# jglaser/metadynamics-plugin

Hardware: AMD Instinct MI355X
Metric: particle_cv_evals_per_s (higher is better)
Workload: dtype f32; 1 GPU; 1xMI355X: 10^6 particles, 2 lamellar CVs (8 Fourier modes each), 256^2 bias grid, well-tempered; particles_per_gpu=1000000, particles_global=1000000, n_cv=2, modes_per_cv=8, grid=256x256, stride=1, fast_trig=1, fast_trig_library_default=1, driver=host, mode=single

## Files before the change

### metadynamics-plugin_amd/csrc/fused.hip

```cpp
#include <hip/hip_runtime.h>
#include <hip/hip_ext.h>

#ifdef MTD_STAMPS
__device__ unsigned long long g_stamps[64];
#define MTD_STAMP(slot, cond)                                                   \
    do                                                                          \
        {                                                                       \
        if (cond) g_stamps[slot] = wall_clock64();                              \
        } while (0)
extern "C" int mtd_debug_read_stamps(unsigned long long *host)
    {
    return (int)hipMemcpyFromSymbol(host, HIP_SYMBOL(g_stamps), sizeof(unsigned long long) * 64);
    }
#else
#define MTD_STAMP(slot, cond) do { } while (0)
#endif

#include "lamellar_host.hpp"
#include "metad_host.hpp"
#include "comm_host.hpp"

#include <cstdlib>
#include <cstring>
#include <map>
// ... 181 lines not shown
        grid_first_pass_sums_256(c, blockIdx.x, sums, s_red);
        MTD_STAMP(20, blockIdx.x == 0 && threadIdx.x == 0);
        }
    else if (wave != 0 && N)
        {
        lam_force_store<S4, NCV, FF_U>(a, out, first, stride, s_wcoef, R);
        if (GROUPS > 1) lam_force_store<S4, NCV, FF_U>(a, out, first1, stride, s_wcoef, R1);
        MTD_STAMP(29, blockIdx.x == n_grid_blocks && threadIdx.x == 64);
        }

    if (blockIdx.x == 0 && wave == 0) publish_step(c, s_chain, deposit, nullptr, COMM ? &ck : nullptr);
    }

template<typename S4, bool FAST>
__global__ __launch_bounds__(FF_THREADS) void k_fused_force_general(const LamKArgs a, const S4 *__restrict__ postype, const ForcePtrs out,
                                                            const unsigned int N, const double two_over_n, const MetadCfg c,
                                                            const int deposit, const unsigned int n_grid_blocks)
    {
    __shared__ EvalShared sh;
    __shared__ float s_wcoef[MTD_MAX_CV * MTD_MAX_TYPES];
    __shared__ double s_red[16];
    __shared__ ModeTables s_mt;

    load_modes(a, s_mt, true);
    reduce_cv_sources(c, sh.cv, s_red);
    __syncthreads();
    evaluate_bias(c, sh, deposit != 0, true);

    if (blockIdx.x < n_grid_blocks)
        {
        const unsigned int g = blockIdx.x * FF_THREADS + threadIdx.x;
        double s1 = 0.0, s2 = 0.0;
        if (g < c.len)
            {
            const double dV = (c.W * sh.scal) * exp(-gauss_exponent(c, g, sh.cv));
            c.grid_delta[g] = dV;
            unsigned int hd = c.hist_delta[g];
            if (sh.on_grid && g == sh.bin)
                {
                hd += 1;
                c.hist_delta[g] = hd;
                c.sigma_grid_delta[g] += c.det_sigma;
                c.hist_gauss_delta[g] += 1;
                }
            const double R = c.rew[g] + (double)hd;
            c.rew[g] = R;
            s1 = R * dV;
// ... 173 lines not shown
    if (slots)
        {
        if (m->comm) return MTD_ERR_UNSUPPORTED;
        for (unsigned int c = 0; c < set->n_cv; ++c)
            {
            if (slots[c] >= m->cfg.n_cv) return MTD_ERR_INVALID_ARGUMENT;
            k.slot[c] = (unsigned char)slots[c];
            }
        }
    hipStream_t s = (hipStream_t)stream;
    rc = metad_flush(m, s);
    if (rc) return rc;
    ForcePtrs out;
    for (unsigned int c = 0; c < MTD_MAX_CV; ++c) out.f[c] = nullptr;
    for (unsigned int c = 0; c < set->n_cv; ++c)
        {
        if (!d_force[c] && n_particles) return MTD_ERR_INVALID_ARGUMENT;
        out.f[c] = d_force[c];
        }
    const int dep = deposit_due(m, timestep);
    const unsigned int n_grid = dep ? m->cfg.n_gblocks : 0;
    const double two_over_n = 2.0 / (double)n_global;
    const bool fast = lam_fast_trig(k) != 0;
    static const bool force_general = std::getenv("MTD_FUSED_GENERAL") != nullptr;
    CommK ck;
    std::memset(&ck, 0, sizeof(ck));
    if (m->comm)
        {
        if (m->cfg.n_cv > (unsigned int)CHAIN_MAX_CV || force_general) return MTD_ERR_UNSUPPORTED;
        rc = comm_current(m->comm, ck);
        if (rc) return rc;
        }
    if (m->cfg.n_cv <= (unsigned int)CHAIN_MAX_CV && !force_general)
        {
        hipEvent_t ev_start = nullptr, ev_stop = nullptr;
        const bool timed = force_profile_next(ev_start, ev_stop);
        dispatch_s4_fast(dtype, fast, [&](auto s4, auto fast_c)
            {
            using S4 = typename decltype(s4)::type;
            constexpr bool FAST = decltype(fast_c)::value;
            dispatch_count<CHAIN_MAX_CV>(set->n_cv, [&](auto n)
                {
                constexpr int NCV = decltype(n)::value, G = ff_groups<S4, NCV, FAST>::value;
                const unsigned int per_block = FF_STREAM_THREADS * FF_U * G;
                unsigned int fblocks = (n_particles + per_block - 1) / per_block;
                if (fblocks == 0 && n_grid == 0) fblocks = 1;
                const unsigned int grid = n_grid + fblocks;
                dispatch_bool(m->comm != nullptr, [&](auto comm_c)
                    {
                    dispatch_bool(k.ortho != 0, [&](auto ortho_c)
                        {
                        const auto kernel = k_fused_force<S4, NCV, FAST, G, decltype(comm_c)::value, decltype(ortho_c)::value>;
                        if (timed)
                            hipExtLaunchKernelGGL(kernel, dim3(grid), dim3(FF_THREADS), 0, s, ev_start, ev_stop, 0, k, (const S4 *)d_postype, out,
                                                  n_particles, two_over_n, m->cfg, dep, n_grid, ck);
                        else
                            kernel<<<grid, FF_THREADS, 0, s>>>(k, (const S4 *)d_postype, out, n_particles, two_over_n, m->cfg, dep, n_grid, ck);
                        });
                    });
                });
            });
        }
    else
        {
        unsigned int fblocks = lam_force_blocks(n_particles);
        if (n_particles == 0) fblocks = n_grid ? 0 : 1;
        const unsigned int grid = n_grid + fblocks;
        dispatch_s4_fast(dtype, fast, [&](auto s4, auto fast_c)
            {
            using S4 = typename decltype(s4)::type;
            k_fused_force_general<S4, decltype(fast_c)::value><<<grid, FF_THREADS, 0, s>>>(k, (const S4 *)d_postype, out, n_particles, two_over_n,
                                                                                        m->cfg, dep, n_grid);
            });
        }
    MTD_LAUNCH_CHECK();
    m->pending_apply = dep;
    m->w_stale = dep;
    return MTD_SUCCESS;
    }

int mtd_profile_force_begin(unsigned int n_launches)
    {
    std::lock_guard<std::mutex> lock(g_force_profile_mutex);
    ForceProfile &p = g_force_profile;
    for (hipEvent_t e : p.ev) (void)hipEventDestroy(e);
    p.ev.clear();
    p.used = 0;
    for (unsigned int i = 0; i < 2 * n_launches; ++i)
        {
        hipEvent_t e = nullptr;
        MTD_HIP_TRY(hipEventCreate(&e));
        p.ev.push_back(e);
        }
    return MTD_SUCCESS;
// ... 64 lines not shown
```

### metadynamics-plugin_amd/csrc/fused_step.hip

```cpp
#include <hip/hip_runtime.h>

#ifdef MTD_STAMPS
__device__ unsigned long long g_step_stamps[64];
__device__ unsigned long long g_step_block[6][256];
#define MTD_BSTAMP(row) do { g_step_block[row][blockIdx.x] = wall_clock64(); } while (0)
extern "C" int mtd_debug_read_step_blocks(unsigned long long *host)
    {
    return (int)hipMemcpyFromSymbol(host, HIP_SYMBOL(g_step_block), sizeof(unsigned long long) * 6 * 256);
    }
#define MTD_STAMP(slot, cond)                                                   \
    do                                                                          \
        {                                                                       \
        if (cond) g_step_stamps[slot] = wall_clock64();                         \
        } while (0)
extern "C" int mtd_debug_read_step_stamps(unsigned long long *host)
    {
    return (int)hipMemcpyFromSymbol(host, HIP_SYMBOL(g_step_stamps), sizeof(unsigned long long) * 64);
    }
#else
#define MTD_STAMP(slot, cond) do { } while (0)
#define MTD_BSTAMP(row) do { } while (0)
#endif

#include "lamellar_host.hpp"
#include "metad_host.hpp"
#include "comm_host.hpp"

#include <cstdlib>
#include <cstring>

namespace
{

using namespace mtd;

constexpr int FS_THREADS = 1024;
constexpr int FS_WAVES = FS_THREADS / MTD_WAVE;
constexpr int FS_U = 4;
constexpr unsigned int FS_MAX_BLOCKS = 256;
constexpr unsigned int FS_MAIN = (FS_WAVES - 1) * MTD_WAVE;
constexpr unsigned int FS_EXTRA_WAVES = 4;
constexpr unsigned int FS_CHUNK = FS_U * FS_MAIN + FS_EXTRA_WAVES * MTD_WAVE;
constexpr unsigned int FS_LL_WORDS = 2 * (CHAIN_MAX_CV + 2);
constexpr int FS_FIRST_PROBE_SLEEP = 12;
constexpr unsigned int FS_LL_PITCH = 512;
constexpr unsigned int FS_LL_REPLICAS = 8;
constexpr unsigned int FS_LL_REPLICA_WORDS = FS_LL_WORDS * FS_LL_PITCH;

template<int NCV, int U> struct StepRegs
    {
    v2f g0[U / 2], g1[U / 2], g2[U / 2];
    int type[U];
    bool ok[U];
    float f[U][NCV][3];
    };

template<int NCV, bool FAST, int U>
__device__ __forceinline__ void step_cv_sums(const LamKArgs &a, const float *s_coeff, const ModeTables &mt, const StepRegs<NCV, U> &R,
                                             float (&acc)[NCV])
    {
    constexpr int P = U / 2;
// ... 22 lines not shown
                    sum[q] += h.w * ((cs * cs) * 2.0f - (FAST ? 0.99999994f : 1.0f));
                    }
                }
#pragma unroll
            for (int u = 0; u < U; ++u)
                {
                const float w = R.ok[u] ? s_coeff[c * MTD_MAX_TYPES + R.type[u]] : 0.0f;
                acc[c] += w * sum[u / 2][u % 2];
                }
            }
        }
    }

template<int NCV, bool FAST, int U>
__device__ __forceinline__ void step_force_unscaled(const LamKArgs &a, const ModeTables &mt, StepRegs<NCV, U> &R)
    {
#pragma unroll
    for (int c = 0; c < NCV; ++c)
        {
#pragma unroll
        for (int u = 0; u < U; ++u) R.f[u][c][0] = R.f[u][c][1] = R.f[u][c][2] = 0.0f;
        if (c < (int)a.n_cv)
            {
            const unsigned int k1 = a.first[c + 1];
#pragma unroll 4
            for (unsigned int k = a.first[c]; k < k1; ++k)
                {
                const float4 h = mt.h[k];
                const float4 q = mt.q[k];
#pragma unroll
                for (int u = 0; u < U; ++u)
                    {
                    const float s = sin2pi<FAST>(h.x * R.g0[u / 2][u % 2] + h.y * R.g1[u / 2][u % 2] + h.z * R.g2[u / 2][u % 2]);
                    R.f[u][c][0] += q.x * s;
                    R.f[u][c][1] += q.y * s;
                    R.f[u][c][2] += q.z * s;
                    }
                }
            }
        }
    }

template<int NCV> struct ExtraRegs
    {
    float g0, g1, g2;
    int type;
    bool ok;
    float f[NCV][3];
    };

template<int NCV, bool FAST>
__device__ __forceinline__ void step_cv_sums_one(const LamKArgs &a, const float *s_coeff, const ModeTables &mt, const ExtraRegs<NCV> &X,
                                                 float (&acc)[NCV])
    {
#pragma unroll
    for (int c = 0; c < NCV; ++c)
        if (c < (int)a.n_cv)
            {
            float sum = 0.0f;
            const unsigned int k1 = a.first[c] + a.nact[c];
#pragma unroll 4
            for (unsigned int k = a.first[c]; k < k1; ++k)
                {
                const float4 h = mt.h[k];
                const float cs = cos2pi<FAST>(h.x * X.g0 + h.y * X.g1 + h.z * X.g2);
                sum += cs;
                sum += h.w * ((cs * cs) * 2.0f - (FAST ? 0.99999994f : 1.0f));
                }
            acc[c] += (X.ok ? s_coeff[c * MTD_MAX_TYPES + X.type] : 0.0f) * sum;
            }
    }

template<int NCV, bool FAST>
__device__ __forceinline__ void step_force_unscaled_one(const LamKArgs &a, const ModeTables &mt, ExtraRegs<NCV> &X)
    {
#pragma unroll
    for (int c = 0; c < NCV; ++c)
        {
        X.f[c][0] = X.f[c][1] = X.f[c][2] = 0.0f;
        if (c < (int)a.n_cv)
            {
            const unsigned int k1 = a.first[c + 1];
#pragma unroll 4
            for (unsigned int k = a.first[c]; k < k1; ++k)
                {
                const float4 h = mt.h[k];
                const float4 q = mt.q[k];
                const float sn = sin2pi<FAST>(h.x * X.g0 + h.y * X.g1 + h.z * X.g2);
                X.f[c][0] += q.x * sn;
                X.f[c][1] += q.y * sn;
                X.f[c][2] += q.z * sn;
                }
            }
        }
    }

template<typename S4, int NCV, bool FAST, bool COMM>
__global__ __launch_bounds__(FS_THREADS, 1) void k_fused_step(const LamKArgs a, const S4 *__restrict__ postype, const ForcePtrs out,
                                                           const unsigned int N, const unsigned int chunk, const double two_over_n,
                                                           const MetadCfg c, const int deposit, const unsigned int cells_per_block,
                                                           const CommK lk, const CommK ck)
    {
    typedef typename scalar4_traits<S4>::scalar scalar;
    constexpr int NS = NCV;
    __shared__ ChainResult s_chain;
    __shared__ float s_coeff[MTD_MAX_CV * MTD_MAX_TYPES];
    __shared__ float s_wcoef[MTD_MAX_CV * MTD_MAX_TYPES];
    __shared__ double s_wave[FS_WAVES * NCV];
    __shared__ double s_red[2 * FS_WAVES];
    __shared__ double s_avg[2];

    __shared__ ModeTables s_cvt;
    __shared__ ModeTables s_mt;

    const int wave = threadIdx.x >> 6;
// ... 13 lines not shown
    const unsigned int ix = p0 + FS_U * FS_MAIN + slot0;
    GridPatch patch;
    X.ok = false;
    if (wave == 0)
        {
#pragma unroll
        for (int u = 0; u < FS_U; ++u) R.ok[u] = false;
        patch = chain_prefetch(c);
        }
    else
        {
#pragma unroll
        for (int u = 0; u < FS_U; ++u)
            {
            const unsigned int i = p0 + u * FS_MAIN + slot0;
            R.ok[u] = i < p1;
            if (N) raw.v[u] = postype[R.ok[u] ? i : N - 1];
            }
        X.ok = has_extra && ix < p1;
        if (N && has_extra) raw_x = postype[X.ok ? ix : N - 1];
        }
    load_coeff(a, s_coeff);
    load_modes_cv(a, s_cvt);
    load_modes(a, s_mt, true);
    __syncthreads();

    MTD_STAMP(1, blockIdx.x == 0 && threadIdx.x == 0); MTD_STAMP(17, blockIdx.x == gridDim.x - 1 && threadIdx.x == 0); MTD_STAMP(33, blockIdx.x == 0 && threadIdx.x == 64);
    float acc[NCV];
#pragma unroll
    for (int i = 0; i < NCV; ++i) acc[i] = 0.0f;
    if (wave != 0)
        {
#pragma unroll
        for (int u = 0; u < FS_U; ++u)
            {
            float x0 = 0.0f, x1 = 0.0f, x2 = 0.0f;
            R.type[u] = 0;
            if (N)
                {
                const Particle p = scalar4_traits<S4>::unpack(raw.v[u]);
                project(a, p, x0, x1, x2);
                R.type[u] = p.type;
                }
            R.g0[u / 2][u % 2] = x0;
            R.g1[u / 2][u % 2] = x1;
            R.g2[u / 2][u % 2] = x2;
            }
// ... 391 lines not shown
```

### metadynamics-plugin_amd/csrc/lamellar.hip

```cpp
#include "lamellar_device.hpp"

#include <cmath>
#include <cstdlib>
#include <cstring>

#include "lamellar_host.hpp"

namespace
{

using namespace mtd;

constexpr int CV_THREADS = 512;
constexpr int CV_UNROLL = 4;
constexpr int FORCE_THREADS = 256;
constexpr int FORCE_UNROLL = 2;

int g_fast_trig = 1;

template<typename S4, int NCV, bool FAST>
__global__ __launch_bounds__(CV_THREADS) void k_lamellar_cv_partials(const LamKArgs a, const S4 *__restrict__ postype,
                                                                     const unsigned int N, double *__restrict__ partials)
    {
    __shared__ float s_coeff[MTD_MAX_CV * MTD_MAX_TYPES];
// ... 85 lines not shown
    double v = 0.0;
    unsigned int b = lane;
    for (; b + 7 * MTD_WAVE < n_partials; b += 8 * MTD_WAVE)
        {
        double t[8];
#pragma unroll
        for (int u = 0; u < 8; ++u) t[u] = partials[(size_t)(b + u * MTD_WAVE) * stride + c];
#pragma unroll
        for (int u = 0; u < 8; ++u) v += t[u];
        }
    for (; b < n_partials; b += MTD_WAVE) v += partials[(size_t)b * stride + c];
    v = wave_sum(v);
    if (lane == 0) out[c] = shift + scale * v;
    }

template<typename S4, bool FAST>
__global__ __launch_bounds__(FORCE_THREADS) void k_lamellar_forces(const LamKArgs a, const S4 *__restrict__ postype,
                                                                   const ForcePtrs out, const unsigned int N,
                                                                   const double *__restrict__ d_bias, const double bias_host,
                                                                   const double two_over_n)
    {
    __shared__ float s_wcoef[MTD_MAX_CV * MTD_MAX_TYPES];
    __shared__ ModeTables s_mt;
    load_modes(a, s_mt, true);
    for (unsigned int i = threadIdx.x; i < MTD_MAX_CV * MTD_MAX_TYPES; i += blockDim.x)
        {
        const unsigned int c = i / MTD_MAX_TYPES;
        double b = 0.0;
        if (c < a.n_cv) b = d_bias ? d_bias[c] : bias_host;
        s_wcoef[i] = (float)((double)a.coeff[c][i % MTD_MAX_TYPES] * b * two_over_n);
        }
    __syncthreads();
    lam_force_pass<S4, FAST, FORCE_UNROLL>(a, postype, out, N, blockIdx.x * blockDim.x + threadIdx.x,
                                           gridDim.x * blockDim.x, s_wcoef, s_mt);
    }


unsigned int env_uint(const char *name, unsigned int dflt)
    {
    const char *s = std::getenv(name);
    if (!s || !*s) return dflt;
    long v = std::strtol(s, nullptr, 10);
    return v > 0 ? (unsigned int)v : dflt;
    }

unsigned int cv_blocks(unsigned int N)
    {
// ... 34 lines not shown
    reciprocal_rows(*box, k.B);
    k.ortho = (k.B[0][1] == 0.0 && k.B[0][2] == 0.0 && k.B[1][0] == 0.0 && k.B[1][2] == 0.0 && k.B[2][0] == 0.0 && k.B[2][1] == 0.0)
                  ? 1u : 0u;
    k.n_cv = set->n_cv;
    k.n_modes = set->n_modes;
    k.n_types = set->n_types;
    if (set->trig_mode != MTD_TRIG_DEFAULT && set->trig_mode != MTD_TRIG_HARDWARE && set->trig_mode != MTD_TRIG_ACCURATE)
        return MTD_ERR_INVALID_ARGUMENT;
    k.trig = (unsigned int)set->trig_mode;
    for (unsigned int c = 0; c <= set->n_cv; ++c) k.first[c] = set->first[c];
    for (unsigned int c = 0; c < MTD_MAX_CV; ++c) k.slot[c] = (unsigned char)c;
    const double two_pi = 2.0 * M_PI;
    for (unsigned int m = 0; m < set->n_modes; ++m)
        for (int d = 0; d < 3; ++d)
            {
            const float hv = (float)set->hkl[m][d];
            const float qv = (float)(two_pi * (set->hkl[m][0] * k.B[0][d] + set->hkl[m][1] * k.B[1][d] + set->hkl[m][2] * k.B[2][d]));
            if (d == 0) { k.h[m].x = hv; k.q[m].x = qv; }
            if (d == 1) { k.h[m].y = hv; k.q[m].y = qv; }
            if (d == 2) { k.h[m].z = hv; k.q[m].z = qv; }
            }
    for (unsigned int c = 0; c < set->n_cv; ++c)
        for (unsigned int t = 0; t < set->n_types; ++t) k.coeff[c][t] = (float)set->coeff[c][t];
    static const bool fold = env_uint("MTD_LAM_FOLD_HARMONICS", 1) != 0;
    for (unsigned int c = 0; c < set->n_cv; ++c)
        {
        bool folded[MTD_MAX_MODES] = {false};
        for (unsigned int m = set->first[c]; fold && m < set->first[c + 1]; ++m)
            {
            if (folded[m] || k.h[m].w != 0.0f) continue;
            const int *hm = set->hkl[m];
            if (hm[0] == 0 && hm[1] == 0 && hm[2] == 0) continue;
            for (unsigned int j = set->first[c]; j < set->first[c + 1]; ++j)
                {
                const int *hj = set->hkl[j];
                if (j != m && !folded[j] && k.h[j].w == 0.0f && hj[0] == 2 * hm[0] && hj[1] == 2 * hm[1] && hj[2] == 2 * hm[2])
                    {
                    k.h[m].w = 1.0f;
                    folded[j] = true;
                    break;
                    }
                }
            }
        unsigned int n = 0;
        for (unsigned int m = set->first[c]; m < set->first[c + 1]; ++m)
            if (!folded[m]) k.corder[set->first[c] + n++] = (unsigned char)m;
        k.nact[c] = (unsigned char)n;
        for (unsigned int m = set->first[c]; m < set->first[c + 1]; ++m)
            if (folded[m]) k.corder[set->first[c] + n++] = (unsigned char)m;
        }
    return MTD_SUCCESS;
    }


unsigned int lam_cv_blocks(unsigned int N) { return cv_blocks(N); }
unsigned int lam_force_blocks(unsigned int N) { return force_blocks(N); }
int lam_fast_trig(const LamKArgs &k)
    {
    if (k.trig == MTD_TRIG_ACCURATE) return 0;
    if (k.trig == MTD_TRIG_DEFAULT && !g_fast_trig) return 0;
    for (unsigned int m = 0; m < k.n_modes; ++m)
        if (std::fabs(k.h[m].x) + std::fabs(k.h[m].y) + std::fabs(k.h[m].z) > 100.0f) return 0;
    return 1;
    }
}

extern "C" {

int mtd_lamellar_set_fast_trig(int enable)
    {
    g_fast_trig = enable ? 1 : 0;
    return MTD_SUCCESS;
// ... 73 lines not shown
    return mtd_reduce_partials(d_scratch, blocks, 2 * n_wave, 2 * n_wave, 1.0, 0.0, d_fourier_modes, stream);
    }

static int lamellar_forces_impl(const mtd_lamellar_set *set, unsigned int n_particles, const void *d_postype,
                                void *const *d_force, int dtype, unsigned int n_global, const double *d_bias,
                                double bias_host, const mtd_box *global_box, mtd_stream_t stream)
    {
    LamKArgs k;
    int rc = fill_kargs(k, set, global_box);
    if (rc) return rc;
    if (!d_force || n_global == 0 || (n_particles && !d_postype)) return MTD_ERR_INVALID_ARGUMENT;
    if (dtype != MTD_F32 && dtype != MTD_F64) return MTD_ERR_INVALID_ARGUMENT;
    ForcePtrs out;
    std::memset(&out, 0, sizeof(out));
    for (unsigned int c = 0; c < set->n_cv; ++c)
        {
        if (!d_force[c] && n_particles) return MTD_ERR_INVALID_ARGUMENT;
        out.f[c] = d_force[c];
        }
    if (n_particles == 0) return MTD_SUCCESS;
    hipStream_t s = (hipStream_t)stream;
    const unsigned int blocks = force_blocks(n_particles);
    const double two_over_n = 2.0 / (double)n_global;
    dispatch_s4_fast(dtype, lam_fast_trig(k) != 0, [&](auto s4, auto fast_c)
        {
        using S4 = typename decltype(s4)::type;
        k_lamellar_forces<S4, decltype(fast_c)::value><<<blocks, FORCE_THREADS, 0, s>>>(k, (const S4 *)d_postype, out, n_particles, d_bias, bias_host,
                                                                                     two_over_n);
        });
    MTD_LAUNCH_CHECK();
    return MTD_SUCCESS;
    }

int mtd_lamellar_forces(const mtd_lamellar_set *set, unsigned int n_particles, const void *d_postype,
                        void *const *d_force, int dtype, unsigned int n_global, const double *d_bias,
                        const mtd_box *global_box, mtd_stream_t stream)
    {
    if (!d_bias) return MTD_ERR_INVALID_ARGUMENT;
    return lamellar_forces_impl(set, n_particles, d_postype, d_force, dtype, n_global, d_bias, 0.0, global_box, stream);
    }

int mtd_compute_sq_forces(unsigned int n_particles, const void *d_postype, void *d_force, int dtype,
                          unsigned int n_wave, const int *lattice_vectors, const double *mode,
                          unsigned int n_types, unsigned int n_global, double bias,
                          const mtd_box *global_box, mtd_stream_t stream)
    {
    if (!lattice_vectors || !mode) return MTD_ERR_INVALID_ARGUMENT;
    if (n_wave == 0 || n_wave > MTD_MAX_MODES || n_types == 0 || n_types > MTD_MAX_TYPES) return MTD_ERR_INVALID_ARGUMENT;
    mtd_lamellar_set set;
    std::memset(&set, 0, sizeof(set));
// ... 14 lines not shown
```

### metadynamics-plugin_amd/csrc/lamellar_device.hpp

```cpp
#pragma once

#include "mtd_device.hpp"

namespace mtd
{

struct LamKArgs
    {
    double B[3][3];
    unsigned int n_cv, n_modes, n_types;
    unsigned int trig;
    unsigned int first[MTD_MAX_CV + 1];
    unsigned char slot[MTD_MAX_CV];
    unsigned int ortho;
    float4 h[MTD_MAX_MODES];
    unsigned char corder[MTD_MAX_MODES];
    unsigned char nact[MTD_MAX_CV];
    float4 q[MTD_MAX_MODES];
    float coeff[MTD_MAX_CV][MTD_MAX_TYPES];
    };

struct ForcePtrs
    {
    void *f[MTD_MAX_CV];
    };

template<bool FAST> __device__ __forceinline__ float cos2pi(float t)
    {
    if (FAST)
        return __builtin_amdgcn_cosf(t);
    else
        return cospif(2.0f * t);
    }

template<bool FAST> __device__ __forceinline__ float sin2pi(float t)
    {
    if (FAST)
        return __builtin_amdgcn_sinf(t);
    else
        return sinpif(2.0f * t);
// ... 11 lines not shown
    {
    if constexpr (ORTHO)
        {
        g0 = (float)(a.B[0][0] * p.x);
        g1 = (float)(a.B[1][1] * p.y);
        g2 = (float)(a.B[2][2] * p.z);
        }
    else
        project(a, p, g0, g1, g2);
    }

__device__ __forceinline__ void load_coeff(const LamKArgs &a, float *s_coeff)
    {
    for (unsigned int i = threadIdx.x; i < MTD_MAX_CV * MTD_MAX_TYPES; i += blockDim.x)
        s_coeff[i] = a.coeff[i / MTD_MAX_TYPES][i % MTD_MAX_TYPES];
    }

struct ModeTables
    {
    float4 h[MTD_MAX_MODES];
    float4 q[MTD_MAX_MODES];
    };

__device__ __forceinline__ void load_modes(const LamKArgs &a, ModeTables &t, const bool with_q)
    {
    for (unsigned int k = threadIdx.x; k < a.n_modes; k += blockDim.x)
        {
        t.h[k] = a.h[k];
        if (with_q) t.q[k] = a.q[k];
        }
    }

__device__ __forceinline__ void load_modes_cv(const LamKArgs &a, ModeTables &t)
    {
    for (unsigned int k = threadIdx.x; k < a.n_modes; k += blockDim.x) t.h[k] = a.h[a.corder[k]];
    }

struct CvTableRegs
    {
    float4 h;
    float c;
    };
__device__ __forceinline__ CvTableRegs stage_cv_tables_request(const LamKArgs &a)
    {
    CvTableRegs r;
    r.h = a.h[min(threadIdx.x, (unsigned int)MTD_MAX_MODES - 1)];
    r.c = (&a.coeff[0][0])[min(threadIdx.x, (unsigned int)(MTD_MAX_CV * MTD_MAX_TYPES) - 1)];
    return r;
    }
__device__ __forceinline__ void stage_cv_tables_store(const CvTableRegs &r, float *s_coeff, ModeTables &t)
    {
    if (threadIdx.x < MTD_MAX_MODES) t.h[threadIdx.x] = r.h;
    if (threadIdx.x < MTD_MAX_CV * MTD_MAX_TYPES) s_coeff[threadIdx.x] = r.c;
    }
inline LamKArgs dense_cv_args(const LamKArgs &k)
    {
    LamKArgs d = k;
    for (unsigned int q = 0; q < k.n_modes && q < MTD_MAX_MODES; ++q)
        {
        d.h[q] = k.h[k.corder[q]];
        d.corder[q] = (unsigned char)q;
        }
    return d;
    }

typedef float v2f __attribute__((ext_vector_type(2)));

template<typename S4, int U> struct RawGroup
    {
    S4 v[U];
    };

template<typename S4, int U>
__device__ __forceinline__ void lam_load_group(const S4 *__restrict__ postype, const unsigned int N, const unsigned int base,
                                               const unsigned int n_threads, RawGroup<S4, U> &g)
    {
    if (N == 0) return;
#pragma unroll
    for (int u = 0; u < U; ++u)
        {
        const unsigned int i = base + u * n_threads;
        g.v[u] = postype[i < N ? i : N - 1];
        }
    }
// ... 83 lines not shown

template<int NCV>
__device__ __forceinline__ void lam_cv_block_reduce(const float (&acc)[NCV], double *s_wave, double *__restrict__ partials,
                                                    const unsigned int block_id)
    {
    const int lane = threadIdx.x & 63;
    const int wave = threadIdx.x >> 6;
    const int n_waves = blockDim.x >> 6;
#pragma unroll
    for (int c = 0; c < NCV; ++c)
        {
        const float v = wave_sum(acc[c]);
        if (lane == 0) s_wave[wave * NCV + c] = (double)v;
        }
    __syncthreads();
    if (threadIdx.x < NCV)
        {
        double r = 0.0;
        for (int w = 0; w < n_waves; ++w) r += s_wave[w * NCV + threadIdx.x];
        partials[block_id * NCV + threadIdx.x] = r;
        }
    }

template<typename S4, bool FAST, int U>
__device__ __forceinline__ void lam_force_pass(const LamKArgs &a, const S4 *__restrict__ postype, const ForcePtrs &out,
                                               const unsigned int N, const unsigned int tid, const unsigned int n_threads,
                                               const float *s_wcoef, const ModeTables &mt)
    {
    typedef typename scalar4_traits<S4>::scalar scalar;
    for (unsigned int base = tid; base < N; base += U * n_threads)
        {
        float g0[U], g1[U], g2[U];
        int type[U];
        bool ok[U];
#pragma unroll
        for (int u = 0; u < U; ++u)
            {
            const unsigned int i = base + u * n_threads;
            ok[u] = i < N;
            const Particle p = scalar4_traits<S4>::load(postype, ok[u] ? i : base);
            project(a, p, g0[u], g1[u], g2[u]);
            type[u] = p.type;
            }
        for (unsigned int c = 0; c < a.n_cv; ++c)
            {
            float fx[U], fy[U], fz[U];
#pragma unroll
            for (int u = 0; u < U; ++u) fx[u] = fy[u] = fz[u] = 0.0f;
            const unsigned int k1 = a.first[c + 1];
#pragma unroll 4
            for (unsigned int k = a.first[c]; k < k1; ++k)
                {
                const float4 h = mt.h[k];
                const float4 q = mt.q[k];
#pragma unroll
                for (int u = 0; u < U; ++u)
                    {
                    const float s = sin2pi<FAST>(h.x * g0[u] + h.y * g1[u] + h.z * g2[u]);
                    fx[u] += q.x * s;
                    fy[u] += q.y * s;
                    fz[u] += q.z * s;
                    }
                }
            S4 *f = (S4 *)out.f[c];
#pragma unroll
            for (int u = 0; u < U; ++u)
                {
                if (ok[u])
                    {
                    const float w = s_wcoef[c * MTD_MAX_TYPES + type[u]];
                    nt_store(scalar4_traits<S4>::make((scalar)(fx[u] * w), (scalar)(fy[u] * w), (scalar)(fz[u] * w), (scalar)0),
                             &f[base + u * n_threads]);
                    }
                }
            }
        }
    }

template<int NCV, int U> struct ForceRegs
    {
    v2f f[U / 2][NCV][3];
    int type[U];
    bool ok[U];
    };

template<typename S4, int U>
__device__ __forceinline__ void lam_force_request(const S4 *__restrict__ postype, const unsigned int N, const unsigned int first,
                                                  const unsigned int stride, RawGroup<S4, U> &raw);
template<typename S4, int NCV, bool FAST, int U, bool ORTHO = false>
__device__ __forceinline__ void lam_force_unscaled_from(const LamKArgs &a, const unsigned int N, const unsigned int first,
                                                        const unsigned int stride, const ModeTables &mt, const RawGroup<S4, U> &raw,
                                                        ForceRegs<NCV, U> &R);

template<typename S4, int NCV, bool FAST, int U>
__device__ __forceinline__ void lam_force_unscaled(const LamKArgs &a, const S4 *__restrict__ postype, const unsigned int N,
                                                   const unsigned int first, const unsigned int stride, const ModeTables &mt,
                                                   ForceRegs<NCV, U> &R)
    {
    RawGroup<S4, U> raw;
    lam_force_request<S4, U>(postype, N, first, stride, raw);
    lam_force_unscaled_from<S4, NCV, FAST, U>(a, N, first, stride, mt, raw, R);
    }

template<typename S4, int U>
__device__ __forceinline__ void lam_force_request(const S4 *__restrict__ postype, const unsigned int N, const unsigned int first,
                                                  const unsigned int stride, RawGroup<S4, U> &raw)
    {
    if (N == 0) return;
#pragma unroll
    for (int u = 0; u < U; ++u)
        {
        const unsigned int i = first + u * stride;
        raw.v[u] = postype[i < N ? i : N - 1];
        }
    }

template<typename S4, int NCV, bool FAST, int U, bool ORTHO>
__device__ __forceinline__ void lam_force_unscaled_from(const LamKArgs &a, const unsigned int N, const unsigned int first,
                                                        const unsigned int stride, const ModeTables &mt, const RawGroup<S4, U> &raw,
                                                        ForceRegs<NCV, U> &R)
    {
    static_assert(U % 2 == 0, "particles are processed in pairs");
    constexpr int P = U / 2;
    v2f g0[P], g1[P], g2[P];
#pragma unroll
    for (int u = 0; u < U; ++u)
        {
        const unsigned int i = first + u * stride;
        R.ok[u] = i < N;
        const Particle p = scalar4_traits<S4>::unpack(raw.v[u]);
        float x0, x1, x2;
        project_o<ORTHO>(a, p, x0, x1, x2);
        g0[u / 2][u % 2] = x0;
        g1[u / 2][u % 2] = x1;
        g2[u / 2][u % 2] = x2;
        R.type[u] = p.type;
        }
#pragma unroll
    for (int c = 0; c < NCV; ++c)
        {
#pragma unroll
        for (int pp = 0; pp < P; ++pp) R.f[pp][c][0] = R.f[pp][c][1] = R.f[pp][c][2] = (v2f)(0.0f);
        if (c < (int)a.n_cv)
            {
            const unsigned int k1 = a.first[c + 1];
#pragma unroll 4
            for (unsigned int k = a.first[c]; k < k1; ++k)
                {
                const float4 h = mt.h[k];
                const float4 q = mt.q[k];
#pragma unroll
                for (int pp = 0; pp < P; ++pp)
                    {
                    const v2f t = h.x * g0[pp] + h.y * g1[pp] + h.z * g2[pp];
                    v2f sn;
                    sn.x = sin2pi<FAST>(t.x);
                    sn.y = sin2pi<FAST>(t.y);
                    R.f[pp][c][0] += q.x * sn;
                    R.f[pp][c][1] += q.y * sn;
                    R.f[pp][c][2] += q.z * sn;
                    }
                }
            }
        }
    }

template<typename S4, int NCV, int U>
__device__ __forceinline__ void lam_force_store(const LamKArgs &a, const ForcePtrs &out, const unsigned int first,
                                                const unsigned int stride, const float *s_wcoef, const ForceRegs<NCV, U> &R)
    {
    typedef typename scalar4_traits<S4>::scalar scalar;
#pragma unroll
    for (int c = 0; c < NCV; ++c)
        {
        if (c < (int)a.n_cv)
            {
            S4 *f = (S4 *)out.f[c];
#pragma unroll
            for (int u = 0; u < U; ++u)
                {
                if (R.ok[u])
                    {
                    const float w = s_wcoef[c * MTD_MAX_TYPES + R.type[u]];
                    const S4 v = scalar4_traits<S4>::make((scalar)(R.f[u / 2][c][0][u % 2] * w), (scalar)(R.f[u / 2][c][1][u % 2] * w),
                                                          (scalar)(R.f[u / 2][c][2][u % 2] * w), (scalar)0);
// ... 9 lines not shown
```

### metadynamics-plugin_amd/csrc/mesh.hip

```cpp
#include "mtd_device.hpp"
#include "comm_host.hpp"
#include "exact_div.hpp"
#include "lamellar_host.hpp"
#include "metad_host.hpp"

#include <algorithm>
#include <cmath>
#include <type_traits>
#include <cstdio>
#include <cstdlib>
#include <cstring>
#include <map>
#include <mutex>
#include <new>
#include <utility>
#include <vector>

namespace
{

using namespace mtd;


struct MeshGeom
// ... 1473 lines not shown
        }
    lds_barrier();

    ForceRegs<NCV, TFC_U> R;
    if (wave == 0)
        {
        double vi[3];
#pragma unroll
        for (int i = 0; i < NCH; ++i) vi[i] = (pre.x[i][0] + pre.x[i][1]) + (pre.x[i][2] + pre.x[i][3]);
        const ChainResult r = chain_wave(c, deposit != 0, true, nullptr, nullptr, false, &pre.patch, pre.patch_ok != 0, true, vi[0], vi[1], vi[2]);
        if (lane == 0) chain_share(s_chain, r);
        if (lane < NCV * MTD_MAX_TYPES)
            {
            const unsigned int cv = lane / MTD_MAX_TYPES;
            const unsigned int gs = cv < a.n_cv ? a.slot[cv] : 0u;
            const double b = gs == 0 ? r.bias[0] : (gs == 1 ? r.bias[1] : r.bias[2]);
            s_wcoef[lane] = (cv < a.n_cv) ? (float)((double)s_wcoef[lane] * b * two_over_n) : 0.0f;
            }
        }
    else
        {
        TileStage<TFC_STREAM_THREADS> st;
        if (work) tile_stage_load<TFC_STREAM_THREADS>(st, sid, n_rows, wxn, s_grow, s_lrow, s_gx, inv);
        if (N) lam_force_unscaled_from<S4, NCV, FAST, TFC_U>(a, N, first, stride, s_mt, raw0, R);
        if (work) tile_stage_store<TFC_STREAM_THREADS>(st, s_inv);
        }
    __syncthreads();

    if (wave != 0 && N)
        {
        lam_force_store<S4, NCV, TFC_U>(a, out, first, stride, s_wcoef, R);
        for (unsigned int f = first + TFC_U * stride; f < N; f += TFC_U * stride)
            {
            lam_force_unscaled<S4, NCV, FAST, TFC_U>(a, postype, N, f, stride, s_mt, R);
            lam_force_store<S4, NCV, TFC_U>(a, out, f, stride, s_wcoef, R);
            }
        }
    if (blockIdx.x < n_grid_blocks) grid_first_pass_256(c, s_chain, blockIdx.x, s_red);
    if (blockIdx.x == 0 && wave == 0) publish_step(c, s_chain, deposit);
    if (!work) return;
    const double bias = mesh_slot == 0 ? s_chain.bias[0] : (mesh_slot == 1 ? s_chain.bias[1] : s_chain.bias[2]);
    const double s = two_over_n * bias;
    while (q < q1)
        {
        const double4 cur = pk;
        const unsigned int qn = q + TF_THREADS;
        pk = packed[min(qn, q_last)];
// ... 2400 lines not shown
    const unsigned int n_lam = set ? set->n_cv : 0u;
    if (!mesh || !m || n_global == 0 || !box || (n_lam && (!slots || !d_force_lamellar))) return MTD_ERR_INVALID_ARGUMENT;
    if (dtype != MTD_F32 && dtype != MTD_F64) return MTD_ERR_INVALID_ARGUMENT;
    if (n_particles == 0 || !d_postype || !d_force_mesh) return MTD_ERR_UNSUPPORTED;
    static const bool off = [] { const char *e = std::getenv("MTD_MESH_FORCE_MERGED"); return e && e[0] == '0'; }();
    if (off || !mesh->tile_path || m->comm) return MTD_ERR_UNSUPPORTED;
    if (m->cfg.n_cv > (unsigned int)mtd::CHAIN_MAX_CV || mesh_slot >= m->cfg.n_cv) return MTD_ERR_UNSUPPORTED;
    if (n_lam > 3 || n_lam >= m->cfg.n_cv) return MTD_ERR_UNSUPPORTED;
    if (n_particles != mesh->n_last) return MTD_ERR_INVALID_ARGUMENT;
    if (m->h_step_err && *m->h_step_err) return MTD_ERR_COMM_TIMEOUT;
    mtd::LamKArgs k;
    int rc = MTD_SUCCESS;
    if (n_lam)
        rc = mtd::fill_kargs(k, set, box);
    else
        std::memset(&k, 0, sizeof(k));
    if (rc) return rc;
    for (unsigned int cv = 0; cv < n_lam; ++cv)
        {
        if (slots[cv] >= m->cfg.n_cv || slots[cv] == mesh_slot) return MTD_ERR_INVALID_ARGUMENT;
        if (!d_force_lamellar[cv]) return MTD_ERR_INVALID_ARGUMENT;
        k.slot[cv] = (unsigned char)slots[cv];
        }
    const int dep = deposit_due(m, timestep);
    const unsigned int n_grid = dep ? m->cfg.n_gblocks : 0;
    const unsigned int blocks = 8 * ((mesh->tg.n_tiles + 7) / 8);
    if (n_grid > blocks) return MTD_ERR_UNSUPPORTED;
    if ((unsigned long long)blocks * TFC_STREAM_THREADS * TFC_U >= (1ull << 31)) return MTD_ERR_UNSUPPORTED;
    MeshGeom g;
    rc = fill_geom(g, mesh, box);
    if (rc) return rc;
    hipStream_t s = (hipStream_t)stream;
    rc = mtd::metad_flush(m, s);
    if (rc) return rc;
    mtd::ForcePtrs out;
    for (unsigned int cv = 0; cv < MTD_MAX_CV; ++cv) out.f[cv] = cv < n_lam ? d_force_lamellar[cv] : nullptr;
    const double two_over_n = 2.0 / (double)n_global;
    const bool fast = n_lam ? mtd::lam_fast_trig(k) != 0 : true;
    const unsigned int n_stream = n_lam ? n_particles : 0u;
#define MTD_LAUNCH_TFC(S4, NCV, FASTV) \
    k_tile_forces_chain<S4, NCV, FASTV><<<blocks, TF_THREADS, 0, s>>>(g, mesh->tg, mesh->lists, mesh->d_mode, mesh->d_packed, mesh->d_inv, (S4 *)d_force_mesh, \
        two_over_n, mesh->n_types, mesh_slot, k, (const S4 *)d_postype, out, n_stream, m->cfg, dep, n_grid)
#define MTD_LAUNCH_TFC_NCV(S4, FASTV) \
    switch (n_lam) { case 0: case 1: MTD_LAUNCH_TFC(S4, 1, FASTV); break; case 2: MTD_LAUNCH_TFC(S4, 2, FASTV); break; default: MTD_LAUNCH_TFC(S4, 3, FASTV); break; }
    if (dtype == MTD_F32)
        {
        if (fast) { MTD_LAUNCH_TFC_NCV(float4, true) } else { MTD_LAUNCH_TFC_NCV(float4, false) }
        }
    else
        {
        if (fast) { MTD_LAUNCH_TFC_NCV(double4, true) } else { MTD_LAUNCH_TFC_NCV(double4, false) }
        }
#undef MTD_LAUNCH_TFC_NCV
#undef MTD_LAUNCH_TFC
    MTD_LAUNCH_CHECK();
    m->pending_apply = dep;
    m->w_stale = dep;
    if (dep) mtd::announce_pending_apply(m, s);
    return MTD_SUCCESS;
    }

int mtd_mesh_slab_bytes(const mtd_mesh *m, unsigned int world, size_t *bytes)
    {
    if (!m || !bytes || world == 0 || world > MTD_COMM_MAX_RANKS) return MTD_ERR_INVALID_ARGUMENT;
    if (m->nz % world || m->ny % world) return MTD_ERR_UNSUPPORTED;
// ... 253 lines not shown
```

Measured before the change: 109.7 billion particle-CV-evals/s.

## Fold second-harmonic force modes into sincos terms and reorder modes densely

In the force kernels, a mode is now folded together with its 2h harmonic when that harmonic's amplitude is exactly twice the base amplitude. The pair is evaluated as sin(t)*(4cos(t)+1), a sincos in place of two separate sin calls. A host-side dense_force_args copy reorders the modes so folded ones come first, drops inactive modes, and runs them in separately unrolled loops with compile-time term types. This is meant to cut transcendental count and loop overhead per particle. It adds a per-call host repack of the kernel args and a stricter folding condition on the coefficients.

Measured after the change: 110.2 billion particle-CV-evals/s (median of 4 runs). About the same (+0.4%).

```diff
diff --git a/metadynamics-plugin_amd/csrc/fused.hip b/metadynamics-plugin_amd/csrc/fused.hip
--- a/metadynamics-plugin_amd/csrc/fused.hip
+++ b/metadynamics-plugin_amd/csrc/fused.hip
@@ -227,7 +227,7 @@
     __shared__ double s_red[16];
     __shared__ ModeTables s_mt;
 
-    load_modes(a, s_mt, true);
+    load_modes_force(a, s_mt);
     reduce_cv_sources(c, sh.cv, s_red);
     __syncthreads();
     evaluate_bias(c, sh, deposit != 0, true);
@@ -447,6 +447,7 @@
     const unsigned int n_grid = dep ? m->cfg.n_gblocks : 0;
     const double two_over_n = 2.0 / (double)n_global;
     const bool fast = lam_fast_trig(k) != 0;
+    const LamKArgs kf = dense_force_args(k);
     static const bool force_general = std::getenv("MTD_FUSED_GENERAL") != nullptr;
     CommK ck;
     std::memset(&ck, 0, sizeof(ck));
@@ -477,10 +478,10 @@
                         {
                         const auto kernel = k_fused_force<S4, NCV, FAST, G, decltype(comm_c)::value, decltype(ortho_c)::value>;
                         if (timed)
-                            hipExtLaunchKernelGGL(kernel, dim3(grid), dim3(FF_THREADS), 0, s, ev_start, ev_stop, 0, k, (const S4 *)d_postype, out,
+                            hipExtLaunchKernelGGL(kernel, dim3(grid), dim3(FF_THREADS), 0, s, ev_start, ev_stop, 0, kf, (const S4 *)d_postype, out,
                                                   n_particles, two_over_n, m->cfg, dep, n_grid, ck);
                         else
-                            kernel<<<grid, FF_THREADS, 0, s>>>(k, (const S4 *)d_postype, out, n_particles, two_over_n, m->cfg, dep, n_grid, ck);
+                            kernel<<<grid, FF_THREADS, 0, s>>>(kf, (const S4 *)d_postype, out, n_particles, two_over_n, m->cfg, dep, n_grid, ck);
                         });
                     });
                 });
@@ -494,7 +495,7 @@
         dispatch_s4_fast(dtype, fast, [&](auto s4, auto fast_c)
             {
             using S4 = typename decltype(s4)::type;
-            k_fused_force_general<S4, decltype(fast_c)::value><<<grid, FF_THREADS, 0, s>>>(k, (const S4 *)d_postype, out, n_particles, two_over_n,
+            k_fused_force_general<S4, decltype(fast_c)::value><<<grid, FF_THREADS, 0, s>>>(kf, (const S4 *)d_postype, out, n_particles, two_over_n,
                                                                                         m->cfg, dep, n_grid);
             });
         }
diff --git a/metadynamics-plugin_amd/csrc/fused_step.hip b/metadynamics-plugin_amd/csrc/fused_step.hip
--- a/metadynamics-plugin_amd/csrc/fused_step.hip
+++ b/metadynamics-plugin_amd/csrc/fused_step.hip
@@ -37,6 +37,7 @@
 constexpr int FS_THREADS = 1024;
 constexpr int FS_WAVES = FS_THREADS / MTD_WAVE;
 constexpr int FS_U = 4;
+constexpr int FS_UF = 2, FS_UP = 2;
 constexpr unsigned int FS_MAX_BLOCKS = 256;
 constexpr unsigned int FS_MAIN = (FS_WAVES - 1) * MTD_WAVE;
 constexpr unsigned int FS_EXTRA_WAVES = 4;
@@ -105,21 +106,18 @@
         for (int u = 0; u < U; ++u) R.f[u][c][0] = R.f[u][c][1] = R.f[u][c][2] = 0.0f;
         if (c < (int)a.n_cv)
             {
-            const unsigned int k1 = a.first[c + 1];
-#pragma unroll 4
-            for (unsigned int k = a.first[c]; k < k1; ++k)
-                {
-                const float4 h = mt.h[k];
-                const float4 q = mt.q[k];
+            lam_force_modes<FS_UF, FS_UP>(a, mt, c, [&](const float4 h, const float4 q, auto term) __attribute__((always_inline))
+                {
 #pragma unroll
                 for (int u = 0; u < U; ++u)
                     {
-                    const float s = sin2pi<FAST>(h.x * R.g0[u / 2][u % 2] + h.y * R.g1[u / 2][u % 2] + h.z * R.g2[u / 2][u % 2]);
+                    const float s = lam_force_term<FAST, decltype(term)::value>(
+                        h.x * R.g0[u / 2][u % 2] + h.y * R.g1[u / 2][u % 2] + h.z * R.g2[u / 2][u % 2], q.w);
                     R.f[u][c][0] += q.x * s;
                     R.f[u][c][1] += q.y * s;
                     R.f[u][c][2] += q.z * s;
                     }
-                }
+                });
             }
         }
     }
@@ -163,17 +161,13 @@
         X.f[c][0] = X.f[c][1] = X.f[c][2] = 0.0f;
         if (c < (int)a.n_cv)
             {
-            const unsigned int k1 = a.first[c + 1];
-#pragma unroll 4
-            for (unsigned int k = a.first[c]; k < k1; ++k)
-                {
-                const float4 h = mt.h[k];
-                const float4 q = mt.q[k];
-                const float sn = sin2pi<FAST>(h.x * X.g0 + h.y * X.g1 + h.z * X.g2);
+            lam_force_modes<FS_UF, FS_UP>(a, mt, c, [&](const float4 h, const float4 q, auto term) __attribute__((always_inline))
+                {
+                const float sn = lam_force_term<FAST, decltype(term)::value>(h.x * X.g0 + h.y * X.g1 + h.z * X.g2, q.w);
                 X.f[c][0] += q.x * sn;
                 X.f[c][1] += q.y * sn;
                 X.f[c][2] += q.z * sn;
-                }
+                });
             }
         }
     }
@@ -233,7 +227,7 @@
         }
     load_coeff(a, s_coeff);
     load_modes_cv(a, s_cvt);
-    load_modes(a, s_mt, true);
+    load_modes_force(a, s_mt);
     __syncthreads();
 
     MTD_STAMP(1, blockIdx.x == 0 && threadIdx.x == 0); MTD_STAMP(17, blockIdx.x == gridDim.x - 1 && threadIdx.x == 0); MTD_STAMP(33, blockIdx.x == 0 && threadIdx.x == 64);
diff --git a/metadynamics-plugin_amd/csrc/lamellar.hip b/metadynamics-plugin_amd/csrc/lamellar.hip
--- a/metadynamics-plugin_amd/csrc/lamellar.hip
+++ b/metadynamics-plugin_amd/csrc/lamellar.hip
@@ -131,7 +131,7 @@
     {
     __shared__ float s_wcoef[MTD_MAX_CV * MTD_MAX_TYPES];
     __shared__ ModeTables s_mt;
-    load_modes(a, s_mt, true);
+    load_modes_force(a, s_mt);
     for (unsigned int i = threadIdx.x; i < MTD_MAX_CV * MTD_MAX_TYPES; i += blockDim.x)
         {
         const unsigned int c = i / MTD_MAX_TYPES;
@@ -212,7 +212,7 @@
             }
     for (unsigned int c = 0; c < set->n_cv; ++c)
         for (unsigned int t = 0; t < set->n_types; ++t) k.coeff[c][t] = (float)set->coeff[c][t];
-    static const bool fold = env_uint("MTD_LAM_FOLD_HARMONICS", 1) != 0;
+    static const bool fold = [] { const char *e = std::getenv("MTD_LAM_FOLD_HARMONICS"); return !(e && e[0] == '0'); }();
     for (unsigned int c = 0; c < set->n_cv; ++c)
         {
         bool folded[MTD_MAX_MODES] = {false};
@@ -224,9 +224,11 @@
             for (unsigned int j = set->first[c]; j < set->first[c + 1]; ++j)
                 {
                 const int *hj = set->hkl[j];
-                if (j != m && !folded[j] && k.h[j].w == 0.0f && hj[0] == 2 * hm[0] && hj[1] == 2 * hm[1] && hj[2] == 2 * hm[2])
+                if (j != m && !folded[j] && k.h[j].w == 0.0f && hj[0] == 2 * hm[0] && hj[1] == 2 * hm[1] && hj[2] == 2 * hm[2]
+                    && k.q[j].x == 2.0f * k.q[m].x && k.q[j].y == 2.0f * k.q[m].y && k.q[j].z == 2.0f * k.q[m].z)
                     {
                     k.h[m].w = 1.0f;
+                    k.q[m].w = 4.0f;
                     folded[j] = true;
                     break;
                     }
@@ -238,6 +240,13 @@
         k.nact[c] = (unsigned char)n;
         for (unsigned int m = set->first[c]; m < set->first[c + 1]; ++m)
             if (folded[m]) k.corder[set->first[c] + n++] = (unsigned char)m;
+        unsigned int nf = 0;
+        for (unsigned int i = 0; i < k.nact[c]; ++i)
+            if (k.h[k.corder[set->first[c] + i]].w != 0.0f) k.forder[set->first[c] + nf++] = k.corder[set->first[c] + i];
+        k.nfold[c] = (unsigned char)nf;
+        for (unsigned int i = 0; i < k.nact[c]; ++i)
+            if (k.h[k.corder[set->first[c] + i]].w == 0.0f) k.forder[set->first[c] + nf++] = k.corder[set->first[c] + i];
+        for (unsigned int i = k.nact[c]; set->first[c] + i < set->first[c + 1]; ++i) k.forder[set->first[c] + i] = k.corder[set->first[c] + i];
         }
     return MTD_SUCCESS;
     }
@@ -357,10 +366,11 @@
     hipStream_t s = (hipStream_t)stream;
     const unsigned int blocks = force_blocks(n_particles);
     const double two_over_n = 2.0 / (double)n_global;
+    const LamKArgs kf = dense_force_args(k);
     dispatch_s4_fast(dtype, lam_fast_trig(k) != 0, [&](auto s4, auto fast_c)
         {
         using S4 = typename decltype(s4)::type;
-        k_lamellar_forces<S4, decltype(fast_c)::value><<<blocks, FORCE_THREADS, 0, s>>>(k, (const S4 *)d_postype, out, n_particles, d_bias, bias_host,
+        k_lamellar_forces<S4, decltype(fast_c)::value><<<blocks, FORCE_THREADS, 0, s>>>(kf, (const S4 *)d_postype, out, n_particles, d_bias, bias_host,
                                                                                      two_over_n);
         });
     MTD_LAUNCH_CHECK();
diff --git a/metadynamics-plugin_amd/csrc/lamellar_device.hpp b/metadynamics-plugin_amd/csrc/lamellar_device.hpp
--- a/metadynamics-plugin_amd/csrc/lamellar_device.hpp
+++ b/metadynamics-plugin_amd/csrc/lamellar_device.hpp
@@ -1,6 +1,8 @@
 #pragma once
 
 #include "mtd_device.hpp"
+
+#include <type_traits>
 
 namespace mtd
 {
@@ -16,6 +18,8 @@
     float4 h[MTD_MAX_MODES];
     unsigned char corder[MTD_MAX_MODES];
     unsigned char nact[MTD_MAX_CV];
+    unsigned char forder[MTD_MAX_MODES];
+    unsigned char nfold[MTD_MAX_CV];
     float4 q[MTD_MAX_MODES];
     float coeff[MTD_MAX_CV][MTD_MAX_TYPES];
     };
@@ -73,12 +77,13 @@
     float4 q[MTD_MAX_MODES];
     };
 
-__device__ __forceinline__ void load_modes(const LamKArgs &a, ModeTables &t, const bool with_q)
+__device__ __forceinline__ void load_modes_force(const LamKArgs &a, ModeTables &t)
     {
     for (unsigned int k = threadIdx.x; k < a.n_modes; k += blockDim.x)
         {
-        t.h[k] = a.h[k];
-        if (with_q) t.q[k] = a.q[k];
+        const unsigned int m = a.forder[k];
+        t.h[k] = a.h[m];
+        t.q[k] = a.q[m];
         }
     }
 
@@ -111,6 +116,31 @@
         {
         d.h[q] = k.h[k.corder[q]];
         d.corder[q] = (unsigned char)q;
+        }
+    return d;
+    }
+
+inline LamKArgs dense_force_args(const LamKArgs &k)
+    {
+    LamKArgs d = k;
+    unsigned int n = 0;
+    for (unsigned int c = 0; c < k.n_cv && c < MTD_MAX_CV; ++c)
+        {
+        d.first[c] = n;
+        for (unsigned int i = 0; i < k.nact[c] && n < MTD_MAX_MODES; ++i, ++n)
+            {
+            const unsigned int m = k.forder[k.first[c] + i];
+            d.h[n] = k.h[m];
+            d.q[n] = k.q[m];
+            d.forder[n] = d.corder[n] = (unsigned char)n;
+            }
+        }
+    for (unsigned int c = k.n_cv; c <= MTD_MAX_CV; ++c) d.first[c] = n;
+    d.n_modes = n;
+    for (unsigned int m = n; m < MTD_MAX_MODES; ++m)
+        {
+        d.h[m] = d.q[m] = make_float4(0.0f, 0.0f, 0.0f, 0.0f);
+        d.forder[m] = d.corder[m] = 0;
         }
     return d;
     }
@@ -240,6 +270,62 @@
         }
     }
 
+enum { LAM_TERM_PLAIN = 0, LAM_TERM_FOLDED = 1, LAM_TERM_BLEND = 2 };
+
+template<bool FAST> __device__ __forceinline__ void sincos2pi(const float t, float &s, float &c)
+    {
+    if (FAST)
+        {
+        s = __builtin_amdgcn_sinf(t);
+        c = __builtin_amdgcn_cosf(t);
+        }
+    else
+        sincospif(2.0f * t, &s, &c);
+    }
+
+template<bool FAST, int TERM> __device__ __forceinline__ float lam_force_term(const float t, const float w4)
+    {
+    if (TERM == LAM_TERM_PLAIN) return sin2pi<FAST>(t);
+    float s, c;
+    sincos2pi<FAST>(t, s, c);
+    return s * ((TERM == LAM_TERM_FOLDED ? 4.0f : w4) * c + 1.0f);
+    }
+template<bool FAST, int TERM> __device__ __forceinline__ v2f lam_force_term(const v2f t, const float w4)
+    {
+    v2f s;
+    if (TERM == LAM_TERM_PLAIN)
+        {
+        s.x = sin2pi<FAST>(t.x);
+        s.y = sin2pi<FAST>(t.y);
+        return s;
+        }
+    float s0, s1, c0, c1;
+    sincos2pi<FAST>(t.x, s0, c0);
+    sincos2pi<FAST>(t.y, s1, c1);
+    v2f c;
+    s.x = s0;
+    s.y = s1;
+    c.x = c0;
+    c.y = c1;
+    return s * ((TERM == LAM_TERM_FOLDED ? 4.0f : w4) * c + 1.0f);
+    }
+
+template<int UF = 4, int UP = 4, typename F>
+__device__ __forceinline__ void lam_force_modes(const LamKArgs &a, const ModeTables &mt, const int c, F &&body)
+    {
+    const unsigned int k0 = a.first[c], k1 = k0 + a.nact[c];
+#ifdef MTD_LAM_FORCE_BLEND
+#pragma unroll UF
+    for (unsigned int k = k0; k < k1; ++k) body(mt.h[k], mt.q[k], std::integral_constant<int, LAM_TERM_BLEND>());
+#else
+    const unsigned int kf = k0 + a.nfold[c];
+#pragma unroll UF
+    for (unsigned int k = k0; k < kf; ++k) body(mt.h[k], mt.q[k], std::integral_constant<int, LAM_TERM_FOLDED>());
+#pragma unroll UP
+    for (unsigned int k = kf; k < k1; ++k) body(mt.h[k], mt.q[k], std::integral_constant<int, LAM_TERM_PLAIN>());
+#endif
+    }
+
 template<typename S4, bool FAST, int U>
 __device__ __forceinline__ void lam_force_pass(const LamKArgs &a, const S4 *__restrict__ postype, const ForcePtrs &out,
                                                const unsigned int N, const unsigned int tid, const unsigned int n_threads,
@@ -265,21 +351,17 @@
             float fx[U], fy[U], fz[U];
 #pragma unroll
             for (int u = 0; u < U; ++u) fx[u] = fy[u] = fz[u] = 0.0f;
-            const unsigned int k1 = a.first[c + 1];
-#pragma unroll 4
-            for (unsigned int k = a.first[c]; k < k1; ++k)
-                {
-                const float4 h = mt.h[k];
-                const float4 q = mt.q[k];
+            lam_force_modes(a, mt, c, [&](const float4 h, const float4 q, auto term) __attribute__((always_inline))
+                {
 #pragma unroll
                 for (int u = 0; u < U; ++u)
                     {
-                    const float s = sin2pi<FAST>(h.x * g0[u] + h.y * g1[u] + h.z * g2[u]);
+                    const float s = lam_force_term<FAST, decltype(term)::value>(h.x * g0[u] + h.y * g1[u] + h.z * g2[u], q.w);
                     fx[u] += q.x * s;
                     fy[u] += q.y * s;
                     fz[u] += q.z * s;
                     }
-                }
+                });
             S4 *f = (S4 *)out.f[c];
 #pragma unroll
             for (int u = 0; u < U; ++u)
@@ -305,7 +387,7 @@
 template<typename S4, int U>
 __device__ __forceinline__ void lam_force_request(const S4 *__restrict__ postype, const unsigned int N, const unsigned int first,
                                                   const unsigned int stride, RawGroup<S4, U> &raw);
-template<typename S4, int NCV, bool FAST, int U, bool ORTHO = false>
+template<typename S4, int NCV, bool FAST, int U, bool ORTHO = false, int UF = 4, int UP = 4>
 __device__ __forceinline__ void lam_force_unscaled_from(const LamKArgs &a, const unsigned int N, const unsigned int first,
                                                         const unsigned int stride, const ModeTables &mt, const RawGroup<S4, U> &raw,
                                                         ForceRegs<NCV, U> &R);
@@ -333,7 +415,7 @@
         }
     }
 
-template<typename S4, int NCV, bool FAST, int U, bool ORTHO>
+template<typename S4, int NCV, bool FAST, int U, bool ORTHO, int UF, int UP>
 __device__ __forceinline__ void lam_force_unscaled_from(const LamKArgs &a, const unsigned int N, const unsigned int first,
                                                         const unsigned int stride, const ModeTables &mt, const RawGroup<S4, U> &raw,
                                                         ForceRegs<NCV, U> &R)
@@ -361,24 +443,18 @@
         for (int pp = 0; pp < P; ++pp) R.f[pp][c][0] = R.f[pp][c][1] = R.f[pp][c][2] = (v2f)(0.0f);
         if (c < (int)a.n_cv)
             {
-            const unsigned int k1 = a.first[c + 1];
-#pragma unroll 4
-            for (unsigned int k = a.first[c]; k < k1; ++k)
-                {
-                const float4 h = mt.h[k];
-                const float4 q = mt.q[k];
+            lam_force_modes<UF, UP>(a, mt, c, [&](const float4 h, const float4 q, auto term) __attribute__((always_inline))
+                {
 #pragma unroll
                 for (int pp = 0; pp < P; ++pp)
                     {
                     const v2f t = h.x * g0[pp] + h.y * g1[pp] + h.z * g2[pp];
-                    v2f sn;
-                    sn.x = sin2pi<FAST>(t.x);
-                    sn.y = sin2pi<FAST>(t.y);
+                    const v2f sn = lam_force_term<FAST, decltype(term)::value>(t, q.w);
                     R.f[pp][c][0] += q.x * sn;
                     R.f[pp][c][1] += q.y * sn;
                     R.f[pp][c][2] += q.z * sn;
                     }
-                }
+                });
             }
         }
     }
diff --git a/metadynamics-plugin_amd/csrc/mesh.hip b/metadynamics-plugin_amd/csrc/mesh.hip
--- a/metadynamics-plugin_amd/csrc/mesh.hip
+++ b/metadynamics-plugin_amd/csrc/mesh.hip
@@ -1519,7 +1519,10 @@
         {
         TileStage<TFC_STREAM_THREADS> st;
         if (work) tile_stage_load<TFC_STREAM_THREADS>(st, sid, n_rows, wxn, s_grow, s_lrow, s_gx, inv);
-        if (N) lam_force_unscaled_from<S4, NCV, FAST, TFC_U>(a, N, first, stride, s_mt, raw0, R);
+        {
+            constexpr int UF = (FAST && NCV <= 2) ? 4 : 2;
+            if (N) lam_force_unscaled_from<S4, NCV, FAST, TFC_U, false, UF, 4>(a, N, first, stride, s_mt, raw0, R);
+            }
         if (work) tile_stage_store<TFC_STREAM_THREADS>(st, s_inv);
         }
     __syncthreads();
@@ -3966,6 +3969,7 @@
         if (!d_force_lamellar[cv]) return MTD_ERR_INVALID_ARGUMENT;
         k.slot[cv] = (unsigned char)slots[cv];
         }
+    const mtd::LamKArgs kf = mtd::dense_force_args(k);
     const int dep = deposit_due(m, timestep);
     const unsigned int n_grid = dep ? m->cfg.n_gblocks : 0;
     const unsigned int blocks = 8 * ((mesh->tg.n_tiles + 7) / 8);
@@ -3984,7 +3988,7 @@
     const unsigned int n_stream = n_lam ? n_particles : 0u;
 #define MTD_LAUNCH_TFC(S4, NCV, FASTV) \
     k_tile_forces_chain<S4, NCV, FASTV><<<blocks, TF_THREADS, 0, s>>>(g, mesh->tg, mesh->lists, mesh->d_mode, mesh->d_packed, mesh->d_inv, (S4 *)d_force_mesh, \
-        two_over_n, mesh->n_types, mesh_slot, k, (const S4 *)d_postype, out, n_stream, m->cfg, dep, n_grid)
+        two_over_n, mesh->n_types, mesh_slot, kf, (const S4 *)d_postype, out, n_stream, m->cfg, dep, n_grid)
 #define MTD_LAUNCH_TFC_NCV(S4, FASTV) \
     switch (n_lam) { case 0: case 1: MTD_LAUNCH_TFC(S4, 1, FASTV); break; case 2: MTD_LAUNCH_TFC(S4, 2, FASTV); break; default: MTD_LAUNCH_TFC(S4, 3, FASTV); break; }
     if (dtype == MTD_F32)
```
